# landrumb/ParlayANN

Measured on AMD Instinct MI355X. Metric: QPS @ recall@10>=0.95, SIFT-1M d=128 beam=64; achieved HBM GB/s vs roofline, higher is better.
Workload: dtype f16; 1 GPU; SIFT-1M-shaped batched beam search: 1000000x128 integer-valued fp32->f16 base, 10000 queries/step/GPU, beam=64 k=10 cut=1.35 start=0, prebuilt Vamana R=64 L=128 alpha=1.15 x2 passes (built on device); n=1000000, d=128, nq_per_gpu=10000, beam=64, k=10, parallelism=query-sharded x1, index replicated, no collective

## Files before the change

### parlayann_amd/csrc/api.hip

```cpp
#include <algorithm>
#include <chrono>
#include <cmath>
#include <cstring>
#include <mutex>
#include <vector>

#include "grouped_plan.h"
#include "host_staging.h"
#include "pann_internal.h"
#include "quant_device.h"

namespace pann {

static thread_local std::string g_err;
void set_error(const std::string& s) { g_err = s; }
int hip_fail(hipError_t e, const char* what) {
  g_err = std::string(what) + ": " + hipGetErrorString(e);
  return PANN_ERR_HIP;
}

constexpr size_t kAllocSlack = 4096;

int Workspace::ensure(size_t need) {
  if (need <= bytes) return PANN_OK;
// ... 440 lines not shown
uint64_t pann_index_size(const pann_index* idx) { return idx ? idx->ix.n : 0; }
uint32_t pann_index_dims(const pann_index* idx) { return idx ? idx->ix.d : 0; }
uint32_t pann_index_max_degree(const pann_index* idx) { return idx ? idx->ix.max_deg : 0; }
int pann_index_device(const pann_index* idx) { return idx ? idx->device : -1; }

int pann_index_set_exact_float_order(pann_index* idx, int on) {
  if (int rc = check_idx(idx, "pann_index_set_exact_float_order")) return rc;
  DeviceIndex& ix = idx->ix;
  const bool is_float = ix.dtype == PANN_F32 || ix.dtype == PANN_F16 || ix.dtype == PANN_BF16;
  if (on && is_float) { ix.exact = 1; ix.lpc = 4; ix.nch = ix.pstride / 64; }
  else { ix.exact = 0; choose_point_layout(ix.dbytes, &ix.lpc, &ix.nch); }
  return PANN_OK;
}

int pann_index_reserve_dropped(pann_index* idx, uint32_t cap) {
  if (int rc = check_idx(idx, "pann_index_reserve_dropped")) return rc;
  if (cap > (1u << 30)) { set_error("pann_index_reserve_dropped: capacity out of range"); return PANN_ERR_BAD_ARG; }
  if (cap > idx->dcap) idx->dcap = (cap + 63) / 64 * 64;
  return PANN_OK;
}
uint32_t pann_index_dropped_capacity(const pann_index* idx) { return idx ? idx->dcap : 0; }

int pann_index_set_graph(pann_index* idx, const uint32_t* graph) {
  if (int rc = check_idx(idx, "pann_index_set_graph")) return rc;
  if (!graph) { set_error("pann_index_set_graph: null graph"); return PANN_ERR_BAD_ARG; }
  DeviceGuard g(idx->device);
  return upload_graph_rows(idx, graph, idx->ix.n, nullptr);
}

int pann_index_update_rows(pann_index* idx, const uint32_t* row_ids, const uint32_t* rows, uint64_t m) {
  if (int rc = check_idx(idx, "pann_index_update_rows")) return rc;
  if (m && (!row_ids || !rows)) { set_error("pann_index_update_rows: null argument"); return PANN_ERR_BAD_ARG; }
  for (uint64_t i = 0; i < m; i++)
    if (row_ids[i] >= idx->ix.n) { set_error("ERROR: graph index out of range"); return PANN_ERR_BAD_ARG; }
  DeviceGuard g(idx->device);
  return upload_graph_rows(idx, rows, m, row_ids);
}

int pann_index_clear_graph(pann_index* idx) {
  if (int rc = check_idx(idx, "pann_index_clear_graph")) return rc;
  DeviceGuard g(idx->device);
  PANN_HIP(hipMemsetAsync(idx->ix.graph, 0xFF, (size_t)idx->ix.n * idx->ix.gstride * 4, idx->stream));
  if (idx->ix.gcode) PANN_HIP(hipMemsetAsync(idx->ix.gcode, 0xFF, (size_t)idx->ix.n * idx->ix.gstride * 2, idx->stream));
  PANN_HIP(hipStreamSynchronize(idx->stream));
  return PANN_OK;
}

int64_t pann_index_get_option(const pann_index* idx, const char* name) {
  if (!idx || !name) return -1;
  const std::string nm = name;
  if (nm == "forest_group") return idx->ix.forest_group;
  if (nm == "gt_pieces") return idx->gt_pieces;
  if (nm == "delete_range_keys") return idx->delete_range_keys;
  if (nm == "locality_order") return idx->ix.cell ? 1 : 0;
  if (nm == "filter_codes") return idx->ix.codes_valid ? 1 : 0;
  if (nm == "pinned_bytes") return (int64_t)(idx->pin_in.bytes + idx->pin_out.bytes);
  return -1;
}

int pann_index_set_stream(pann_index* idx, void* stream, int use_private) {
  if (int rc = check_idx(idx, "pann_index_set_stream")) return rc;
  DeviceGuard g(idx->device);
  PANN_HIP(hipStreamSynchronize(idx->stream));
  idx->stream = use_private ? idx->own_stream : (hipStream_t)stream;
  return PANN_OK;
}

int pann_index_set_option(pann_index* idx, const char* name, int64_t value) {
  if (int rc = check_idx(idx, "pann_index_set_option")) return rc;
  const std::string nm = name ? name : "";
  if (value < 0 || value > 0x7FFFFFFF) { set_error("pann_index_set_option: value out of range"); return PANN_ERR_BAD_ARG; }
  if (nm == "forest_group") idx->ix.forest_group = (uint32_t)value;
  else if (nm == "gt_pieces") idx->gt_pieces = (uint32_t)value;
  else if (nm == "delete_range_keys") idx->delete_range_keys = (uint32_t)value;
  else if (nm == "locality_pivots") { idx->locality_pivots = std::max<uint32_t>(2, std::min<uint32_t>((uint32_t)value, 65536)); idx->ix.cell = nullptr; idx->cells_state = idx->cells_state < 0 ? idx->cells_state : 0; }
  else if (nm == "locality_groups") { idx->locality_groups = (uint32_t)std::min<int64_t>(value, 4096); idx->ix.cell = nullptr; idx->cells_state = idx->cells_state < 0 ? idx->cells_state : 0; }
  else if (nm == "locality_order") {
    idx->ix.cell = nullptr;
    idx->ix.cell_min_batch = value == 2 ? 64u : 4096u;
    idx->cells_state = value ? ((idx->cell_buf.buf && idx->cells_state == 1) ? 1 : 0) : -2;
    if (idx->cells_state == 1) idx->ix.cell = idx->cell_buf.as<uint32_t>();
  }
  else if (nm == "filter_codes") {
    idx->ix.codes_valid = 0;
    idx->codes_state = value ? (idx->ix.rank16 ? 1 : 0) : -2;
  }
  else { set_error("pann_index_set_option: unknown option '" + nm + "'"); return PANN_ERR_BAD_ARG; }
  return PANN_OK;
}

int pann_index_get_graph(pann_index* idx, uint32_t* graph_out) {
  if (int rc = check_idx(idx, "pann_index_get_graph")) return rc;
  if (!graph_out) { set_error("pann_index_get_graph: null output"); return PANN_ERR_BAD_ARG; }
  DeviceGuard g(idx->device);
  DeviceIndex& ix = idx->ix;
  const size_t row_bytes = (size_t)(ix.max_deg + 1) * 4;
  const uint64_t slice = std::max<uint64_t>(1, (256ull << 20) / row_bytes);
  for (uint64_t r0 = 0; r0 < ix.n; r0 += slice) {
    const uint64_t cnt = std::min(slice, ix.n - r0);
    if (int rc = idx->graph_slab.ensure(cnt * row_bytes)) return rc;
    hipLaunchKernelGGL(graph_to_host_layout_kernel, dim3((uint32_t)cnt), dim3(64), 0, idx->stream,
                       ix.graph + r0 * (uint64_t)ix.gstride, idx->graph_slab.as<uint32_t>(), cnt, ix.max_deg, ix.gstride);
    PANN_HIP(hipGetLastError());
    PANN_HIP(hipMemcpyAsync(graph_out + r0 * (ix.max_deg + 1), idx->graph_slab.buf, cnt * row_bytes, hipMemcpyDeviceToHost, idx->stream));
    PANN_HIP(hipStreamSynchronize(idx->stream));
  }
  return PANN_OK;
}


static int masked_search_checks(const pann_index* idx, const PointFilter& F, uint64_t nq, const pann_query_params* qp, const pann_search_out* out) {
  if ((int64_t)out->out_k > qp->beam) { set_error("pann_batch_search_masked: out_k larger than the beam"); return PANN_ERR_BAD_ARG; }
  if (F.mode == MASK_BITMAP) { if (int rc = filter_checks(idx, "pann_batch_search_masked", F, nq)) return rc; }
  if (out->out_k > 64) { set_error("pann_batch_search_masked: out_k > 64 is not supported"); return PANN_ERR_UNSUPPORTED; }
  return PANN_OK;
}

static int search_common_checks(pann_index* idx, uint64_t nq, const pann_query_params* qp, const pann_search_out* out) {
  if (int rc = check_idx(idx, "pann_batch_search")) return rc;
  if (!qp || !out) { set_error("pann_batch_search: null params/out"); return PANN_ERR_BAD_ARG; }
  if (int rc = k_beam_check(qp)) return rc;
  (void)nq;
  return PANN_OK;
}

static int batch_search_dev_impl(pann_index* idx, const void* d_queries, const uint32_t* d_query_ids,
                                 uint64_t nq, uint64_t q_stride_bytes, const uint32_t* d_starts,
// ... 1897 lines not shown
```

### parlayann_amd/csrc/beam_search.hip

```cpp
#include <cstdio>
#include <cstdlib>
#include <vector>

#include "pann_device.h"

namespace pann {

#ifndef PANN_GU
#define PANN_GU 4
#endif
#ifndef PANN_GU_B128
#define PANN_GU_B128(LPC, NCH1) 4
#endif
#ifndef PANN_MINWAVES
#define PANN_MINWAVES 1
#endif
#ifndef PANN_B128_PAIR_CODES
#define PANN_B128_PAIR_CODES 1
#endif
#ifndef PANN_B64_PREFETCH
#define PANN_B64_PREFETCH 1
#endif
#ifndef PANN_MINWAVES_B64
#define PANN_MINWAVES_B64 7
// ... 69 lines not shown
}
template <bool HASH_LDS>
__device__ __forceinline__ void hstore(uint32_t* H, uint32_t s, uint32_t v) {
  if constexpr (HASH_LDS) H[s] = v;
  else __hip_atomic_store(H + s, v, __ATOMIC_RELAXED, PANN_PRIVATE_SCOPE);
}
template <bool HASH_LDS>
__device__ __forceinline__ void hsync() {
  if constexpr (!HASH_LDS) __builtin_amdgcn_s_waitcnt(0);
  PANN_WSYNC();
}

__device__ __forceinline__ uint32_t lower_bound_lds(const uint64_t* A, uint32_t n, uint64_t key) {
  uint32_t lo = 0, hi = n;
  while (lo < hi) {
    uint32_t mid = (lo + hi) >> 1;
    if (A[mid] < key) lo = mid + 1; else hi = mid;
  }
  return lo;
}

__device__ __forceinline__ uint32_t split_lds_index(uint32_t s, uint32_t hb) {
  return hb == 1 ? (s >> 1) : hb == 3 ? s : (s >> 2) * 3 + (s & 3);
}
struct LdsPart { uint8_t* base; uint32_t nslots; uint32_t p24; };
__device__ __forceinline__ uint32_t lds_part_load(const LdsPart& L, uint32_t i) {
  if (L.p24) {
    const uint32_t lo = reinterpret_cast<const uint16_t*>(L.base)[i];
    const uint32_t hi = (L.base + 2 * L.nslots)[i];
    return lo | (hi << 16);
  }
  return reinterpret_cast<const uint32_t*>(L.base)[i];
}
__device__ __forceinline__ void lds_part_store(const LdsPart& L, uint32_t i, uint32_t a) {
  if (L.p24) {
    reinterpret_cast<uint16_t*>(L.base)[i] = (uint16_t)a;
    (L.base + 2 * L.nslots)[i] = (uint8_t)(a >> 16);
  } else {
    reinterpret_cast<uint32_t*>(L.base)[i] = a;
  }
}
__device__ __forceinline__ void lds_part_clear(const LdsPart& L, int lane) {
  if (L.p24) {
    uint32_t* w = reinterpret_cast<uint32_t*>(L.base);
    for (uint32_t i = lane; i < (3 * L.nslots) / 4; i += PANN_WAVE) w[i] = 0xFFFFFFFFu;
  } else {
    uint32_t* w = reinterpret_cast<uint32_t*>(L.base);
    for (uint32_t i = lane; i < L.nslots; i += PANN_WAVE) w[i] = SENTINEL;
  }
}

template <bool HASH_LDS>
__device__ __forceinline__ bool filter_update(uint32_t* H, uint32_t hmask, bool active, uint32_t a, int lane,
                                              uint8_t* T = nullptr, uint32_t hb = 0, LdsPart Lp = LdsPart{nullptr, 0, 0}) {
  const uint32_t s = (uint32_t)hash64_2((uint64_t)a) & hmask;
  uint32_t old, w;
  const uint32_t hm = (1u << hb) - 1u;
  const bool in_hbm = hb != 3 && (s & hm) == hm;
  if constexpr (HASH_LDS) {
    old = active ? H[s] : 0u;
    PANN_WSYNC();
    if (active) H[s] = (uint32_t)lane;
    PANN_WSYNC();
    w = active ? H[s] : (uint32_t)lane;
  } else {
    __builtin_amdgcn_s_waitcnt(0);
    old = 0u;
    if (active) old = in_hbm ? __hip_atomic_load(H + (s >> hb), __ATOMIC_RELAXED, PANN_PRIVATE_SCOPE) : lds_part_load(Lp, split_lds_index(s, hb));
    const uint32_t t = s & 1023u;
    if (active) T[t] = (uint8_t)lane;
    PANN_WSYNC();
    w = active ? (uint32_t)T[t] : (uint32_t)lane;
  }
  uint64_t losers = __ballot(active && w != (uint32_t)lane);
  int prev = -1;
  bool last = true;
  while (losers) {
    const int L = __ffsll((unsigned long long)losers) - 1;
    const uint32_t sL = __builtin_amdgcn_readlane(s, L);
    const uint64_t grp = __ballot(active && s == sL);
    losers &= ~grp;
    if (active && s == sL) {
      const uint64_t below = grp & ((1ull << lane) - 1ull);
      prev = below ? 63 - __clzll((unsigned long long)below) : -1;
      last = (lane == 63) ? true : ((grp >> (lane + 1)) == 0ull);
    }
  }
  const uint32_t a_prev = __shfl(a, prev < 0 ? lane : prev);
  const bool seen = active && (prev >= 0 ? (a_prev == a) : (old == a));
  if constexpr (HASH_LDS) {
    PANN_WSYNC();
    if (active && last) H[s] = a;
    PANN_WSYNC();
  } else {
    if (active && last) {
      if (in_hbm) __hip_atomic_store(H + (s >> hb), a, __ATOMIC_RELAXED, PANN_PRIVATE_SCOPE);
      else lds_part_store(Lp, split_lds_index(s, hb), a);
    }
    PANN_WSYNC();
  }
  return seen;
}

struct FilterUndo { uint32_t s, old; bool wrote; };
__device__ __forceinline__ void code_store(uint8_t* P8, uint32_t* P4, uint32_t s, uint32_t code) {
  const uint32_t sh = (s & 7u) * 4u;
  P8[s] = (uint8_t)code;
  const uint32_t addr = (uint32_t)(uintptr_t)(P4 + (s >> 3));
  asm volatile("ds_mskor_b32 %0, %1, %2" ::"v"(addr), "v"(0xFu << sh), "v"((code >> 8) << sh) : "memory");
}
__device__ __forceinline__ void filter_undo_codes(uint8_t* P8, uint32_t* P4, const FilterUndo& u) {
  if (u.wrote) code_store(P8, P4, u.s, u.old);
  PANN_WSYNC();
}
__device__ __forceinline__ bool filter_update_codes(uint8_t* P8, uint32_t* P4, uint32_t hmask, bool active, uint32_t a, uint32_t code,
                                                    int lane, uint8_t* T, FilterUndo* undo = nullptr) {
  const uint32_t s = (uint32_t)hash64_2((uint64_t)a) & hmask;
  const uint32_t sh = (s & 7u) * 4u;
  uint32_t old = 0x1000u;
  if (active) old = (uint32_t)P8[s] | (((P4[s >> 3] >> sh) & 0xFu) << 8);
  const uint32_t t = s & 1023u;
  if (active) T[t] = (uint8_t)lane;
  PANN_WSYNC();
  const uint32_t w = active ? (uint32_t)T[t] : (uint32_t)lane;
  uint64_t losers = __ballot(active && w != (uint32_t)lane);
  int prev = -1;
  bool last = true;
  while (losers) {
    const int L = __ffsll((unsigned long long)losers) - 1;
    const uint32_t sL = __builtin_amdgcn_readlane(s, L);
    const uint64_t grp = __ballot(active && s == sL);
    losers &= ~grp;
    if (active && s == sL) {
      const uint64_t below = grp & ((1ull << lane) - 1ull);
      prev = below ? 63 - __clzll((unsigned long long)below) : -1;
      last = (lane == 63) ? true : ((grp >> (lane + 1)) == 0ull);
    }
  }
  const uint32_t a_prev = __shfl(a, prev < 0 ? lane : prev);
  const bool seen = active && (prev >= 0 ? (a_prev == a) : (old == code));
  if (undo) { undo->s = s; undo->old = old; undo->wrote = active && last; }
  if (active && last) code_store(P8, P4, s, code);
  PANN_WSYNC();
// ... 384 lines not shown
              }
              const uint64_t lm = __ballot(lost);
              if (lost) {
                const uint32_t at = ndrop + lanes_below(lm, lane);
                if (at < P.dcap) DL[at] = key; else atomicOr(P.status, 2u);
              }
              ndrop = min(ndrop + (uint32_t)__popcll(lm), P.dcap);
            }
            __builtin_amdgcn_s_waitcnt(0);
          }
          { uint64_t* t = F; F = NF; NF = t; uint8_t* tv = Fv; Fv = NFv; NFv = tv; }
          f = f_new;
          c = 0;
          PANN_WSYNC();
        }
      }
      PANN_STAMP(4);
      first = false;
    }

    const size_t qo = (size_t)qi * P.out.out_k;
    if constexpr (MASKED) {
      const uint64_t rkey = R.L[lane];
      const uint64_t fill = __ballot(rkey != KEY_INF);
      if (lane < (int)P.out.out_k) {
        const bool ok = rkey != KEY_INF;
        if (P.out.ids) P.out.ids[qo + lane] = ok ? key_id(rkey) : SENTINEL;
        if (P.out.dists) P.out.dists[qo + lane] = ok ? key_dist(rkey) : __builtin_inff();
      }
      if (lane == 0) {
        if (P.result_count) P.result_count[qi] = min((uint32_t)__popcll(fill), P.out.out_k);
        if (P.allowed_cmps) P.allowed_cmps[qi] = R.cmps;
      }
    } else {
    for (uint32_t j = lane; j < P.out.out_k; j += PANN_WAVE) {
      const bool ok = j < f;
      uint64_t key = 0ull;
      if (ok) key = F[j];
      if (P.out.ids) P.out.ids[qo + j] = ok ? key_id(key) : SENTINEL;
      if (P.out.dists) P.out.dists[qo + j] = ok ? key_dist(key) : __builtin_inff();
    }
    }
    PANN_STAMP_FLUSH(qi);
    if (lane == 0) {
      write_counters(P, qi, f, nvis, dcmps, degsum);
      if constexpr (FILTER) if (P.pruned_cmps) P.pruned_cmps[qi] = pcmps;
    }
    PANN_WSYNC();
    if constexpr (HASH_LDS) break;
    else slot = next_slot(P, lane);
  }
}

template <int DT, int METRIC, int LPC, bool NCH1, int MASKED = MASK_NONE>
__global__ void __launch_bounds__(PANN_WAVE, PANN_MINWAVES_B64) beam_search_b64_kernel(BSParams P) {
  const int lane = threadIdx.x;
  extern __shared__ __align__(16) uint8_t smem[];
  uint64_t* S = reinterpret_cast<uint64_t*>(smem);
  uint64_t* C = S + 64;
  uint8_t* Sv = reinterpret_cast<uint8_t*>(C + P.ccap);
  uint4* qlds = reinterpret_cast<uint4*>(Sv + 64);
  uint32_t* H = reinterpret_cast<uint32_t*>(qlds + (NCH1 ? 0 : P.nch * LPC));
  uint32_t* Pl = reinterpret_cast<uint32_t*>(S);

  const uint32_t hsize = 1u << P.bits, hmask = hsize - 1u;
  const uint32_t beam = P.beam;
  const uint32_t BIG_ORD = f2ord(2147483648.0f);
  const uint32_t qi = P.order ? P.order[blockIdx.x] : blockIdx.x;
  if (blockIdx.x >= P.prio_start) __builtin_amdgcn_s_setprio(3);

  for (uint32_t i = lane; i < hsize; i += PANN_WAVE) H[i] = SENTINEL;
  const int64_t self = P.query_ids ? (int64_t)P.query_ids[qi] : -1;
  const uint8_t* qrow = P.query_ids ? P.points + (uint64_t)self * P.pstride : P.queries + (uint64_t)qi * P.qstride;
  QReg<DT> qreg{};
  load_query<DT, LPC, NCH1>(qrow, P.dbytes, P.nch, qreg, qlds, lane);
  PANN_WSYNC();

  uint32_t f = 0, c = 0, nvis = 0, dcmps = P.nstarts, degsum = 0, ndrop = 0;
  uint64_t fkey = KEY_INF;
  uint32_t fflag = 0;
  uint64_t* DL = P.dropped + (size_t)qi * P.dcap;
  [[maybe_unused]] MaskedList R{reinterpret_cast<uint64_t*>(smem + P.rl_off), P.out.out_k ? KEY_INF : 0ull, 0u};
  [[maybe_unused]] const uint32_t thr_lane = P.out.out_k ? P.out.out_k - 1u : 0u;
  [[maybe_unused]] MaskSrc M{};
  if constexpr (MASKED) { M = mask_src<MASKED>(P, qi); R.L[lane] = KEY_INF; }
  PANN_STAMP_BEGIN();

  {
    const bool act = lane < (int)P.nstarts;
    const uint32_t a = act ? P.starts[(size_t)qi * P.starts_stride + lane] : 0u;
    (void)filter_update<true>(H, hmask, act, a, lane);
    [[maybe_unused]] uint32_t aword = 0u;
    if constexpr (MASKED) if (act) aword = mask_word<MASKED>(M, a);
    if (act) Pl[lane] = a;
    PANN_WSYNC();
    if constexpr (MASKED)
      c = gather_distances_masked<DT, METRIC, LPC, NCH1, 4, MASKED>(P, qreg, qlds, Pl, P.nstarts, 0xFFFFFFFFu, C, c, lane,
                                                            masked_note(act, (uint32_t)lane, a), aword, M, R, thr_lane);
    else
    c = gather_distances<DT, METRIC, LPC, NCH1, 4>(P, qreg, qlds, Pl, P.nstarts, 0xFFFFFFFFu, C, c, lane);
    PANN_WSYNC();
  }

  uint32_t pref_id = SENTINEL, pref_row = SENTINEL;
  bool first = true;
  for (;;) {
    bool do_merge = first;
    if (!first) {
      const uint64_t um = __ballot(lane < (int)f && fflag == 0);
      if (um == 0ull || nvis >= P.limit) break;
      const int cur_idx = __ffsll((unsigned long long)um) - 1;
      const bool more_unvisited = (um & (um - 1)) != 0ull;
      PANN_STAMP(0);
      const uint64_t cur_key = readlane64(fkey, cur_idx);
      const uint32_t cur = key_id(cur_key);
      if (lane == cur_idx) fflag = 1;
      if (lane == 0 && P.out.visited_cap) record_visit(P, qi, nvis, cur_key);
      nvis++;
      uint32_t cutoff_ord = BIG_ORD;
      if (f == beam) cutoff_ord = (uint32_t)(readlane64(fkey, (int)f - 1) >> 32);

      asm volatile("s_waitcnt vmcnt(0)" : "+v"(pref_row));
      const bool pref_hit = PANN_B64_PREFETCH && (pref_id == cur);
      const uint32_t pref_val = pref_row;
      pref_id = SENTINEL;
      if (PANN_B64_PREFETCH) {
        const uint64_t rest = um & (um - 1);
        if (rest) {
          pref_id = key_id(readlane64(fkey, __ffsll((unsigned long long)rest) - 1));
          const uint32_t* np = P.graph + (size_t)pref_id * P.gstride + min((uint32_t)lane, P.gstride - 1);
          asm volatile("global_load_dword %0, %1, off" : "=v"(pref_row) : "v"(np));
        }
      }

      const uint32_t* row = P.graph + (size_t)cur * P.gstride;
      for (uint32_t i0 = 0; i0 < P.gstride; i0 += PANN_WAVE) {
        const uint32_t i = i0 + lane;
        uint32_t a = SENTINEL;
        if (i0 == 0 && pref_hit) { if (i < P.gstride) a = pref_val; }
        else if (i < P.gstride) a = row[i];
        const bool act = (a != SENTINEL) && (i < P.degree_limit);
        const uint64_t am = __ballot(act);
        PANN_STAMP(1);
        if (am == 0ull) break;
        degsum += __popcll(am);
        const bool seen = filter_update<true>(H, hmask, act, a, lane);
        const bool keep = act && !seen && ((int64_t)a != self);
        const uint64_t km = __ballot(keep);
        const uint32_t m = __popcll(km);
        [[maybe_unused]] uint32_t aword = 0u;
        if constexpr (MASKED) if (keep) aword = mask_word<MASKED>(M, a);
        const uint32_t mypos = lanes_below(km, lane);
        if (keep) Pl[mypos] = a;
        dcmps += m;
        PANN_WSYNC();
        PANN_STAMP(2);
        if constexpr (MASKED) {
          if (m) c = gather_distances_masked<DT, METRIC, LPC, NCH1, PANN_GU, MASKED>(P, qreg, qlds, Pl, m, cutoff_ord, C, c, lane,
                                                                             masked_note(keep, mypos, a), aword, M, R, thr_lane);
        } else {
        if (m) c = gather_distances<DT, METRIC, LPC, NCH1, PANN_GU>(P, qreg, qlds, Pl, m, cutoff_ord, C, c, lane);
        }
        PANN_WSYNC();
        PANN_STAMP(3);
      }
      const bool skip = (c == 0) || (P.skip_enabled && c < beam / 8 && more_unvisited);
      do_merge = !skip;
    }
    if (do_merge) {
      const uint32_t f_old = f;
      const bool track = P.cut_enabled && !first;
      uint32_t lt = 0;
      for (uint32_t c0 = 0; c0 < c; c0 += PANN_WAVE) {
        const uint32_t cc = min(c - c0, (uint32_t)PANN_WAVE);
        const uint64_t ckey = (lane < (int)cc) ? C[c0 + lane] : KEY_INF;
        const bool fl = lane < (int)f;
        uint32_t myp = 0, rank_c = 0, below_f = 0;
        uint64_t live_mask = 0;
        const uint64_t vmask = __ballot(fl);
        const uint32_t cid = (uint32_t)ckey, fid = (uint32_t)fkey;
        for (uint32_t i = 0; i < cc; i++) {
          const uint64_t kk = readlane64(ckey, (int)i);
          const uint32_t kid = (uint32_t)kk;
          const bool g = kk < fkey;
          const uint64_t gtm = __ballot(g);
          const uint64_t eqm = __ballot(fid == kid);
          const uint64_t dupm = __ballot(cid == kid) & ((1ull << i) - 1ull);
          if (eqm == 0ull && dupm == 0ull) {
            live_mask |= 1ull << i;
            if (lane == (int)i) myp = f - (uint32_t)__popcll(gtm & vmask);
            rank_c += (kk < ckey) ? 1u : 0u;
            below_f += g ? 1u : 0u;
          }
        }
        const uint32_t nvalid = __popcll(live_mask);
        const bool clive = (lane < (int)cc) && ((live_mask >> lane) & 1ull);
        const uint32_t cpos = rank_c + myp, fpos = (uint32_t)lane + below_f;
        if (clive && cpos < beam) {
          uint32_t flag = 0u;
          for (uint32_t t = 0; t < ndrop; t++)
            flag |= (__hip_atomic_load(DL + t, __ATOMIC_RELAXED, PANN_PRIVATE_SCOPE) == ckey) ? 2u : 0u;
          S[cpos] = ckey; Sv[cpos] = (uint8_t)flag;
        }
        if (fl && fpos < beam) { S[fpos] = fkey; Sv[fpos] = (uint8_t)fflag; }
        if (track) {
          const bool lost = fl && fflag == 1u && fpos >= beam;
          const uint64_t lm = __ballot(lost);
          if (lost) {
            const uint32_t at = ndrop + lt + lanes_below(lm, lane);
            if (at < P.dcap) DL[at] = fkey; else atomicOr(P.status, 2u);
          }
          lt += __popcll(lm);
        }
        PANN_WSYNC();
        f = min(f + nvalid, beam);
        fkey = (lane < (int)f) ? S[lane] : KEY_INF;
        fflag = (lane < (int)f) ? (uint32_t)Sv[lane] : 0u;
        PANN_WSYNC();
      }
      uint32_t f_new = f;
      if (!first && P.cut_enabled && f_new > P.k) {
        const float dk = key_dist(readlane64(fkey, (int)P.k));
        const float thr = (float)(P.cut * (double)dk);
        const uint64_t thr_key = (uint64_t)f2ord(thr) << 32;
        const uint32_t ub = __popcll(__ballot(lane < (int)f_new && fkey <= thr_key));
        f_new = max(ub, f_old);
      }
      if (f_new == beam) {
        ndrop = 0;
      } else if (track) {
        const bool lost = lane >= (int)f_new && lane < (int)f && fflag == 1u;
        const uint64_t lm = __ballot(lost);
        if (lost) {
          const uint32_t at = ndrop + lt + lanes_below(lm, lane);
          if (at < P.dcap) DL[at] = fkey; else atomicOr(P.status, 2u);
        }
        lt += __popcll(lm);
        ndrop = min(ndrop + lt, P.dcap);
        if (lt) __builtin_amdgcn_s_waitcnt(0);
      }
      f = f_new;
      if (lane >= (int)f) { fkey = KEY_INF; fflag = 0u; }
      c = 0;
    }
    PANN_STAMP(4);
    first = false;
  }
  asm volatile("s_waitcnt vmcnt(0)" : "+v"(pref_row));

  const size_t qo = (size_t)qi * P.out.out_k;
  if constexpr (MASKED) {
    const uint64_t rkey = R.L[lane];
    const uint64_t fill = __ballot(rkey != KEY_INF);
    if (lane < (int)P.out.out_k) {
      const bool ok = rkey != KEY_INF;
      if (P.out.ids) P.out.ids[qo + lane] = ok ? key_id(rkey) : SENTINEL;
      if (P.out.dists) P.out.dists[qo + lane] = ok ? key_dist(rkey) : __builtin_inff();
    }
    if (lane == 0) {
      if (P.result_count) P.result_count[qi] = min((uint32_t)__popcll(fill), P.out.out_k);
      if (P.allowed_cmps) P.allowed_cmps[qi] = R.cmps;
    }
  } else
  if (lane < (int)P.out.out_k) {
    const bool ok = lane < (int)f;
    if (P.out.ids) P.out.ids[qo + lane] = ok ? key_id(fkey) : SENTINEL;
    if (P.out.dists) P.out.dists[qo + lane] = ok ? key_dist(fkey) : __builtin_inff();
  }
  PANN_STAMP_FLUSH(qi);
  if (lane == 0) write_counters(P, qi, f, nvis, dcmps, degsum);
}

template <int DT, int METRIC, int LPC, bool NCH1, bool HASH_LDS, bool CODES = false>
__global__ void __launch_bounds__(PANN_WAVE) beam_search_b128_kernel(BSParams P) {
  static_assert(!CODES || HASH_LDS, "the code table lives in LDS");
  constexpr int RB = 2;
  const int lane = threadIdx.x;
  extern __shared__ __align__(16) uint8_t smem[];
  uint64_t* S = reinterpret_cast<uint64_t*>(smem);
// ... 273 lines not shown
  PANN_STAMP_FLUSH(qi);

  const size_t qo = (size_t)qi * P.out.out_k;
#pragma unroll
  for (int r = 0; r < RB; r++) {
    const uint32_t j = lane + 64 * r;
    if (j < P.out.out_k) {
      const bool ok = j < f;
      if (P.out.ids) P.out.ids[qo + j] = ok ? key_id(fkey[r]) : SENTINEL;
      if (P.out.dists) P.out.dists[qo + j] = ok ? key_dist(fkey[r]) : __builtin_inff();
    }
  }
  if (lane == 0) write_counters(P, qi, f, nvis, dcmps, degsum);
  if constexpr (HASH_LDS) {
    break;
  } else {
    PANN_WSYNC();
    slot = next_slot(P, lane, slot);
  }
  }
}


void choose_point_layout(uint32_t dbytes, uint32_t* lpc, uint32_t* nch) {
  const uint32_t r64 = (dbytes + 63) / 64 * 64;
  if (const char* f = ab_env("PANN_FORCE_LPC")) {
    const uint32_t l = (uint32_t)atoi(f);
    if ((l == 4 || l == 8 || l == 16) && r64 % (l * 16) == 0 && r64 / (l * 16) > 1) { *lpc = l; *nch = r64 / (l * 16); return; }
  }
  if (r64 == 128) { *lpc = 8; *nch = 1; return; }
  if (r64 == 256) { *lpc = 16; *nch = 1; return; }
  if (r64 == 512) { *lpc = 32; *nch = 1; return; }
  if (r64 % 256 == 0) { *lpc = 16; *nch = r64 / 256; return; }
  if (r64 % 128 == 0) { *lpc = 8; *nch = r64 / 128; return; }
  *lpc = 4; *nch = r64 / 64;
}

static uint32_t filter_bits(int64_t beam) {
  double l = std::ceil(std::log2((double)beam * (double)beam)) - 2.0;
  int b = (int)l;
  return (uint32_t)(b < 10 ? 10 : b);
}

struct Plan {
  uint32_t bits, bcap, ccap, deg_eff, dcap, lds_bytes; bool hash_lds; uint32_t slots; bool b64; bool b128;
  bool b128_codes;
  bool b128_hbm;
  uint32_t hsplit;
  uint32_t p24;
  bool filter; uint32_t sk_lds_off;
  uint32_t rl_off;
  bool masked;
  bool by_labels;
};

constexpr bool masked_b64_fits(int dtype, uint32_t lpc, bool nch1) { return !(lpc == 8 && nch1) && !(dtype == PANN_BF16 && !nch1); }

static Plan make_plan(const DeviceIndex& ix, const SearchArgs& a) {
  Plan p;
  p.bits = filter_bits(a.beam);
  const uint32_t beam = (uint32_t)a.beam;
  p.bcap = (std::max<uint32_t>(beam, a.nstarts) + 63) / 64 * 64;
  int64_t dl = std::min<int64_t>(std::max<int64_t>(a.degree_limit, 0), (int64_t)ix.max_deg);
  p.deg_eff = (uint32_t)dl;
  p.ccap = (std::max<uint32_t>(beam / 8 + p.deg_eff, a.nstarts) + 63) / 64 * 64;
  p.dcap = std::max<uint32_t>(a.dcap, 64);
  const bool nch1 = layout_query_in_registers(ix);
  size_t fixed = (size_t)p.bcap * 8 * 2 + (size_t)p.ccap * 8 + (size_t)p.bcap * 2 +
                 (size_t)p.ccap * 2 + (nch1 ? 0 : (size_t)ix.nch * ix.lpc * 16);
  size_t hbytes = (size_t)4 << p.bits;
  p.hash_lds = (hbytes <= 16384) && (fixed + hbytes <= 64 * 1024);
  p.lds_bytes = (uint32_t)(fixed + (p.hash_lds ? hbytes : 1024));
  p.slots = 256 * 8;
  p.filter = a.filter != 0; p.sk_lds_off = 0;
  p.masked = a.masked != MASK_NONE; p.by_labels = a.masked == MASK_LABELS; p.rl_off = 0;
  const bool masked_b64 = p.hash_lds && p.bcap == 64 && masked_b64_fits(ix.dtype, ix.lpc, nch1);
  if (p.masked && !masked_b64) {
    p.b64 = p.b128 = p.b128_codes = p.b128_hbm = false; p.hsplit = 0; p.p24 = 0;
    p.rl_off = (p.lds_bytes + 15u) & ~15u;
    p.lds_bytes = p.rl_off + 1024;
    return p;
  }
  if (p.filter) {
    p.b64 = p.b128 = p.b128_codes = p.b128_hbm = false; p.hsplit = 0; p.p24 = 0;
    p.sk_lds_off = (p.lds_bytes + 15u) & ~15u;
    p.lds_bytes = p.sk_lds_off + ix.sk_stride;
    return p;
  }
  p.b64 = p.hash_lds && p.bcap == 64;
  if (p.b64) {
    p.ccap = (std::max<uint32_t>(beam / 8 + p.deg_eff, a.nstarts) + 7) / 8 * 8;
    p.lds_bytes = (uint32_t)(64 * 8 + (size_t)p.ccap * 8 + 64 + (nch1 ? 0 : (size_t)ix.nch * ix.lpc * 16) + hbytes);
    if (p.masked) { p.rl_off = (p.lds_bytes + 15u) & ~15u; p.lds_bytes = p.rl_off + 1024; }
  }
  p.b128 = p.hash_lds && p.bcap == 128 && a.nstarts <= 64;
  p.b128_hbm = false;
  p.b128_codes = p.b128 && p.bits == FILTER_CODE_BITS && ix.codes_valid && ix.gcode && ix.rank16 && ix.gstride <= PANN_WAVE;
  if (p.b128_codes) {
    p.ccap = (std::max<uint32_t>(beam / 8 + p.deg_eff, a.nstarts) + 7) / 8 * 8;
    p.hsplit = 0; p.p24 = 0;
    p.lds_bytes = (uint32_t)(128 * 8 + (size_t)p.ccap * 8 + 128 + (nch1 ? 0 : (size_t)ix.nch * ix.lpc * 16) + ((size_t)1 << p.bits) * 3 / 2);
  } else if (p.b128) {
    p.ccap = (std::max<uint32_t>(beam / 8 + p.deg_eff, a.nstarts) + 7) / 8 * 8;
    static const bool force_lds = ab_env("PANN_B128_LDS") != nullptr;
    p.b128_hbm = (hbytes > 8192) && a.nq > 2048 && !force_lds;
    p.hsplit = 0;
    if (p.b128_hbm) {
      static const char* sp = ab_env("PANN_B128_SPLIT");
      p.hsplit = sp ? (uint32_t)atoi(sp) : 1u;
      if (p.hsplit > 3) p.hsplit = 0;
      static const bool no24 = ab_env("PANN_B128_NO24") != nullptr;
      if (p.hsplit == 3 && (no24 || !(ix.n < 0xFFFFFFull))) p.hsplit = 1;
      p.hash_lds = false; p.slots = 256 * 32;
      p.p24 = (p.hsplit && ix.n < 0xFFFFFFull && !no24) ? 1u : 0u;
      hbytes = p.hsplit == 3 ? ((size_t)3 << p.bits)
             : p.hsplit ? (((size_t)1 << p.bits) - ((size_t)1 << (p.bits - p.hsplit))) * (p.p24 ? 3 : 4) : 0;
    }
    p.lds_bytes = (uint32_t)(128 * 8 + (size_t)p.ccap * 8 + 128 + (nch1 ? 0 : (size_t)ix.nch * ix.lpc * 16) + hbytes);
  }
  return p;
}

size_t search_workspace_bytes(const DeviceIndex& ix, const SearchArgs& a) {
  Plan p = make_plan(ix, a);
  size_t need = 256;
  need += (size_t)a.nq * p.dcap * 8;
  if (!p.hash_lds) need += ((size_t)std::min<uint64_t>(a.nq, p.slots) << p.bits) * 4;
  return need;
}

using SearchKernel = void (*)(BSParams);
static hipError_t launch_search(SearchKernel kern, const BSParams& P, const Plan& p, bool persistent, hipStream_t stream) {
  if (p.lds_bytes > 48 * 1024)
    (void)hipFuncSetAttribute(reinterpret_cast<const void*>(kern), hipFuncAttributeMaxDynamicSharedMemorySize, (int)p.lds_bytes);
  const uint32_t grid = persistent ? (uint32_t)std::min<uint64_t>(P.nq, p.slots) : P.nq;
  hipLaunchKernelGGL(kern, dim3(grid), dim3(PANN_WAVE), p.lds_bytes, stream, P);
  return hipGetLastError();
}

template <int DT, int METRIC, int LPC, bool NCH1, int MODE>
static SearchKernel masked_kernel(const Plan& p) {
  if (p.b64) {
    if constexpr (masked_b64_fits(DT, LPC, NCH1)) return beam_search_b64_kernel<DT, METRIC, LPC, NCH1, MODE>;
    else return nullptr;
  }
  if (p.hash_lds) return beam_search_kernel<DT, METRIC, LPC, NCH1, true, false, MODE>;
  return beam_search_kernel<DT, METRIC, LPC, NCH1, false, false, MODE>;
}

template <int DT, int METRIC, int LPC, bool NCH1>
static hipError_t launch_variant(const BSParams& P, const Plan& p, hipStream_t stream) {
  SearchKernel kern;
  if (p.filter) {
    if (p.hash_lds) kern = beam_search_kernel<DT, METRIC, LPC, NCH1, true, true>;
    else kern = beam_search_kernel<DT, METRIC, LPC, NCH1, false, true>;
  } else if (p.masked) {
    kern = p.by_labels ? masked_kernel<DT, METRIC, LPC, NCH1, MASK_LABELS>(p) : masked_kernel<DT, METRIC, LPC, NCH1, MASK_BITMAP>(p);
    if (!kern) return hipErrorInvalidValue;
  } else if (p.b64) {
    kern = beam_search_b64_kernel<DT, METRIC, LPC, NCH1>;
  } else if (p.b128_codes) {
    kern = beam_search_b128_kernel<DT, METRIC, LPC, NCH1, true, true>;
  } else if (p.b128) {
    if (p.b128_hbm) kern = beam_search_b128_kernel<DT, METRIC, LPC, NCH1, false>;
    else kern = beam_search_b128_kernel<DT, METRIC, LPC, NCH1, true>;
  } else if (p.hash_lds) {
    kern = beam_search_kernel<DT, METRIC, LPC, NCH1, true>;
  } else {
    kern = beam_search_kernel<DT, METRIC, LPC, NCH1, false>;
  }
  return launch_search(kern, P, p, !p.hash_lds, stream);
}

template <int DT, int METRIC>
static hipError_t launch_layout(const DeviceIndex& ix, const BSParams& P, const Plan& p, hipStream_t s) {
  if (layout_query_in_registers(ix)) {
    if (ix.lpc == 8) return launch_variant<DT, METRIC, 8, true>(P, p, s);
    if (ix.lpc == 16) return launch_variant<DT, METRIC, 16, true>(P, p, s);
    if (ix.lpc == 32) return launch_variant<DT, METRIC, 32, true>(P, p, s);
  }
  if (ix.lpc == 4) return launch_variant<DT, METRIC, 4, false>(P, p, s);
  if (ix.lpc == 8) return launch_variant<DT, METRIC, 8, false>(P, p, s);
  if (ix.lpc == 16) return launch_variant<DT, METRIC, 16, false>(P, p, s);
  return hipErrorInvalidValue;
}

int launch_beam_search(const DeviceIndex& ix, const SearchArgs& a, void* ws, size_t ws_bytes,
                       hipStream_t stream) {
  if (a.nq == 0) return PANN_OK;
  if (a.nq > 0xFFFFFFF0ull) { set_error("pann_batch_search: nq too large"); return PANN_ERR_BAD_ARG; }
  if (a.beam <= 0 || a.beam > 65536) { set_error("pann_batch_search: beam out of range [1,65536]"); return PANN_ERR_BAD_ARG; }
  if (a.nstarts == 0) {
    set_error("beam search expects at least one start point"); return PANN_ERR_BAD_ARG;
  }
  if ((int64_t)a.nstarts > a.beam) { set_error("pann_batch_search: more start points than beam"); return PANN_ERR_BAD_ARG; }
  if (a.out.out_k > (uint64_t)a.beam) {
    set_error("Error: beam search parameter Q same size or smaller than k"); return PANN_ERR_BAD_ARG;
  }
  if ((a.queries == nullptr) == (a.query_ids == nullptr)) {
    set_error("pann_batch_search: exactly one of queries / query_ids must be given"); return PANN_ERR_BAD_ARG;
  }
  if (a.filter) {
    if (!ix.sketch || !sketch_kind_ok(ix.sk_kind)) { set_error("pann_batch_search_filtered: no sketch attached to the index"); return PANN_ERR_BAD_ARG; }
    if ((a.queries != nullptr) != (a.sketch_queries != nullptr)) {
      set_error("pann_batch_search_filtered: sketch_queries go with queries, and only with them"); return PANN_ERR_BAD_ARG;
    }
    if (a.sketch_queries && (a.sq_stride < sketch_row_bytes(ix.sk_kind, ix.d) || a.sq_stride % 8 != 0 || (uintptr_t)a.sketch_queries % 8 != 0)) {
      set_error("pann_batch_search_filtered: sketch query stride smaller than a sketch row, or rows not 8-byte aligned"); return PANN_ERR_BAD_ARG;
    }
  }
  if (a.masked && a.filter) { set_error("pann_batch_search_masked: the sketch filter has no masked form"); return PANN_ERR_UNSUPPORTED; }
  if (a.masked == MASK_LABELS && (!a.labels || !a.preds || a.pred_stride > 1 || !pred_kind_known(a.pred_kind))) {
    set_error("pann_batch_search_labeled: labels, predicates of a known kind and a predicate stride of 0 or 1 are needed"); return PANN_ERR_BAD_ARG;
// ... 77 lines not shown
```

### parlayann_amd/csrc/pann_internal.h

```cpp
#pragma once
#include <hip/hip_runtime.h>
#include <stdint.h>
#include <stdlib.h>
#include <algorithm>
#include <string>

#include "../../include/pann.h"

namespace pann {

constexpr uint32_t SENTINEL = 0xFFFFFFFFu;

#ifdef PANN_AB
inline const char* ab_env(const char* name) { return getenv(name); }
#else
inline const char* ab_env(const char*) { return nullptr; }
#endif

inline bool is_4bit_dtype(int dtype) { return dtype == PANN_U4 || dtype == PANN_I4; }
inline const char* dtype_name(int dtype) {
  switch (dtype) {
    case PANN_U8: return "PANN_U8"; case PANN_I8: return "PANN_I8"; case PANN_F32: return "PANN_F32"; case PANN_F16: return "PANN_F16";
    case PANN_BF16: return "PANN_BF16"; case PANN_U4: return "PANN_U4"; case PANN_I4: return "PANN_I4";
  }
  return "unknown dtype";
}
inline uint32_t esize_of(int dtype) {
  switch (dtype) { case PANN_U8: case PANN_I8: return 1; case PANN_F16: case PANN_BF16: return 2; case PANN_F32: return 4; }
  return 0;
}
inline bool dtype_known(int dtype) { return esize_of(dtype) != 0 || is_4bit_dtype(dtype); }
inline uint64_t row_bytes_of(int dtype, uint64_t d) { return is_4bit_dtype(dtype) ? (d + 1) / 2 : d * esize_of(dtype); }

struct DeviceIndex {
  uint8_t* points = nullptr;
  uint32_t* graph = nullptr;
  uint64_t n = 0;
  uint32_t d = 0;
  int dtype = 0, metric = 0;
  uint32_t esize = 0;
  uint32_t dbytes = 0;
  uint32_t pstride = 0;
  uint32_t lpc = 0;
  uint32_t nch = 0;
  uint32_t exact = 0;
  uint32_t max_deg = 0;
  uint32_t gstride = 0;
  uint32_t forest_group = 0;
  const uint16_t* rank16 = nullptr;
  uint16_t* gcode = nullptr;
  uint32_t codes_valid = 0;
  const uint32_t* cell = nullptr;
  uint32_t cell_min_batch = 4096;
  const uint8_t* sketch = nullptr;
  uint32_t sk_stride = 0;
  int sk_kind = -1;
  uint32_t sk_as_written = 0;
  const uint32_t* labels = nullptr;
};

inline bool layout_query_in_registers(const DeviceIndex& ix) { return ix.nch == 1 && ix.lpc != 4; }
inline size_t query_lds_bytes(const DeviceIndex& ix) { return layout_query_in_registers(ix) ? 0 : (size_t)ix.nch * ix.lpc * 16; }

enum { MASK_NONE = 0, MASK_BITMAP = 1, MASK_LABELS = 2 };
inline bool pred_kind_known(int kind) { return kind == PANN_PRED_ANY || kind == PANN_PRED_MATCH || kind == PANN_PRED_RANGE; }

struct SearchArgs {
  const uint8_t* queries; uint64_t qstride;
  const uint32_t* query_ids;
  uint64_t nq;
  const uint32_t* starts; uint32_t nstarts;
  int starts_per_query = 0;
  int64_t k, beam, limit, degree_limit; double cut;
  uint32_t dcap = 256;
  const uint32_t* order = nullptr;
  pann_search_out out;
  int filter = 0;
  const uint8_t* sketch_queries = nullptr;
  uint64_t sq_stride = 0;
  uint32_t* pruned_cmps = nullptr;
  int masked = 0;
  const uint32_t* allow = nullptr;
  uint64_t allow_stride = 0;
  uint32_t* result_count = nullptr;
  uint32_t* allowed_cmps = nullptr;
  const uint32_t* labels = nullptr;
  const pann_label_pred* preds = nullptr;
  uint32_t pred_stride = 0;
  int pred_kind = 0;
};

struct PointFilter {
  enum { SHARED, PER_QUERY, TABLE };
  int mode = MASK_NONE, layout = SHARED;
  uint64_t count = 1;
  const uint32_t* allow = nullptr; uint64_t stride = 0;
  const uint32_t* labels = nullptr; int kind = 0; const pann_label_pred* preds = nullptr;
  const uint32_t* group = nullptr; bool dev = false;
  static PointFilter bitmap(const uint32_t* allow, uint64_t stride, uint64_t nq, bool dev) {
    PointFilter f; f.mode = MASK_BITMAP; f.allow = allow; f.stride = stride; f.dev = dev;
    if (stride) { f.layout = PER_QUERY; f.count = nq; }
// ... 184 lines not shown
```

Before: 7.435 million queries/s.

## Add LDS victim cache to skip distance recomputation for hash-evicted candidates in b64 search

Adds a small direct-mapped LDS victim table holding node ids evicted from the visited hash filter in the beam-64 kernel. When a neighbor hits this table while the beam is full, its key is looked up in the frontier or candidate lists and re-inserted without fetching the vector or recomputing the distance. It is on by default via a new index option, and it costs extra LDS per block, possible occupancy loss, and extra per-iteration ballots and readlane loops.

```diff
diff --git a/parlayann_amd/csrc/api.hip b/parlayann_amd/csrc/api.hip
--- a/parlayann_amd/csrc/api.hip
+++ b/parlayann_amd/csrc/api.hip
@@ -516,6 +516,7 @@
   if (nm == "forest_group") return idx->ix.forest_group;
   if (nm == "gt_pieces") return idx->gt_pieces;
   if (nm == "delete_range_keys") return idx->delete_range_keys;
+  if (nm == "b64_seen") return idx->ix.b64_seen;
   if (nm == "locality_order") return idx->ix.cell ? 1 : 0;
   if (nm == "filter_codes") return idx->ix.codes_valid ? 1 : 0;
   if (nm == "pinned_bytes") return (int64_t)(idx->pin_in.bytes + idx->pin_out.bytes);
@@ -537,6 +538,7 @@
   if (nm == "forest_group") idx->ix.forest_group = (uint32_t)value;
   else if (nm == "gt_pieces") idx->gt_pieces = (uint32_t)value;
   else if (nm == "delete_range_keys") idx->delete_range_keys = (uint32_t)value;
+  else if (nm == "b64_seen") idx->ix.b64_seen = value ? 1u : 0u;
   else if (nm == "locality_pivots") { idx->locality_pivots = std::max<uint32_t>(2, std::min<uint32_t>((uint32_t)value, 65536)); idx->ix.cell = nullptr; idx->cells_state = idx->cells_state < 0 ? idx->cells_state : 0; }
   else if (nm == "locality_groups") { idx->locality_groups = (uint32_t)std::min<int64_t>(value, 4096); idx->ix.cell = nullptr; idx->cells_state = idx->cells_state < 0 ? idx->cells_state : 0; }
   else if (nm == "locality_order") {
diff --git a/parlayann_amd/csrc/beam_search.hip b/parlayann_amd/csrc/beam_search.hip
--- a/parlayann_amd/csrc/beam_search.hip
+++ b/parlayann_amd/csrc/beam_search.hip
@@ -145,7 +145,8 @@
 
 template <bool HASH_LDS>
 __device__ __forceinline__ bool filter_update(uint32_t* H, uint32_t hmask, bool active, uint32_t a, int lane,
-                                              uint8_t* T = nullptr, uint32_t hb = 0, LdsPart Lp = LdsPart{nullptr, 0, 0}) {
+                                              uint8_t* T = nullptr, uint32_t hb = 0, LdsPart Lp = LdsPart{nullptr, 0, 0},
+                                              uint32_t* victim = nullptr) {
   const uint32_t s = (uint32_t)hash64_2((uint64_t)a) & hmask;
   uint32_t old, w;
   const uint32_t hm = (1u << hb) - 1u;
@@ -182,6 +183,7 @@
   const uint32_t a_prev = __shfl(a, prev < 0 ? lane : prev);
   const bool seen = active && (prev >= 0 ? (a_prev == a) : (old == a));
   if constexpr (HASH_LDS) {
+    if (victim) *victim = (active && last && old != SENTINEL && old != a) ? old : SENTINEL;
     PANN_WSYNC();
     if (active && last) H[s] = a;
     PANN_WSYNC();
@@ -672,8 +674,12 @@
   }
 }
 
-template <int DT, int METRIC, int LPC, bool NCH1, int MASKED = MASK_NONE>
+enum { B64_SEEN = 3 };
+template <int DT, int METRIC, int LPC, bool NCH1, int MODE = MASK_NONE>
 __global__ void __launch_bounds__(PANN_WAVE, PANN_MINWAVES_B64) beam_search_b64_kernel(BSParams P) {
+  constexpr int MASKED = (MODE == MASK_BITMAP || MODE == MASK_LABELS) ? MODE : MASK_NONE;
+  constexpr int VN = MODE == B64_SEEN ? (int)B64_SEEN_N : 0;
+  static_assert((B64_SEEN_N & (B64_SEEN_N - 1)) == 0 && B64_SEEN_N >= 128, "V: a power of two of whole words per lane");
   const int lane = threadIdx.x;
   extern __shared__ __align__(16) uint8_t smem[];
   uint64_t* S = reinterpret_cast<uint64_t*>(smem);
@@ -686,6 +692,10 @@
   const uint32_t hsize = 1u << P.bits, hmask = hsize - 1u;
   const uint32_t beam = P.beam;
   const uint32_t BIG_ORD = f2ord(2147483648.0f);
+  constexpr uint32_t VSHIFT = VN ? (uint32_t)__builtin_ctz((unsigned)(VN ? VN : 1)) : 0u;
+  [[maybe_unused]] uint16_t* V = reinterpret_cast<uint16_t*>(H + hsize);
+  [[maybe_unused]] bool v_ok = true;
+  if constexpr (VN != 0) for (uint32_t i = lane; i < VN / 2; i += PANN_WAVE) reinterpret_cast<uint32_t*>(V)[i] = 0xFFFFFFFFu;
   const uint32_t qi = P.order ? P.order[blockIdx.x] : blockIdx.x;
   if (blockIdx.x >= P.prio_start) __builtin_amdgcn_s_setprio(3);
 
@@ -764,15 +774,44 @@
         PANN_STAMP(1);
         if (am == 0ull) break;
         degsum += __popcll(am);
-        const bool seen = filter_update<true>(H, hmask, act, a, lane);
-        const bool keep = act && !seen && ((int64_t)a != self);
+        [[maybe_unused]] uint32_t victim = SENTINEL;
+        bool seen;
+        if constexpr (VN != 0) seen = filter_update<true>(H, hmask, act, a, lane, nullptr, 0, LdsPart{nullptr, 0, 0}, &victim);
+        else seen = filter_update<true>(H, hmask, act, a, lane);
+        bool keep = act && !seen && ((int64_t)a != self);
+        if constexpr (VN != 0) {
+          dcmps += __popcll(__ballot(keep));
+          if (f == beam && v_ok && cutoff_ord <= BIG_ORD && c <= PANN_WAVE) {
+            const bool hit = keep && V[a & (VN - 1)] == (uint16_t)(a >> VSHIFT);
+            uint64_t hm = __ballot(hit);
+            if (hm) {
+              const uint64_t pkey = lane < (int)c ? C[lane] : KEY_INF;
+              const uint32_t fid = (uint32_t)fkey, pid = (uint32_t)pkey;
+              while (hm) {
+                const int l = __ffsll((unsigned long long)hm) - 1;
+                hm &= hm - 1;
+                const uint32_t al = __builtin_amdgcn_readlane(a, l);
+                const uint64_t inf = __ballot(fid == al), inc = __ballot(pid == al);
+                uint64_t key = KEY_INF;
+                if (inf) key = readlane64(fkey, __ffsll((unsigned long long)inf) - 1);
+                else if (inc) key = readlane64(pkey, __ffsll((unsigned long long)inc) - 1);
+                if ((uint32_t)(key >> 32) < cutoff_ord) {
+                  if (lane == 0) C[c] = key;
+                  c++;
+                }
+              }
+              keep = keep && !hit;
+            }
+          }
+          if (victim != SENTINEL) V[victim & (VN - 1)] = (uint16_t)(victim >> VSHIFT);
+        }
         const uint64_t km = __ballot(keep);
         const uint32_t m = __popcll(km);
         [[maybe_unused]] uint32_t aword = 0u;
         if constexpr (MASKED) if (keep) aword = mask_word<MASKED>(M, a);
         const uint32_t mypos = lanes_below(km, lane);
         if (keep) Pl[mypos] = a;
-        dcmps += m;
+        if constexpr (VN == 0) dcmps += m;
         PANN_WSYNC();
         PANN_STAMP(2);
         if constexpr (MASKED) {
@@ -845,6 +884,7 @@
         const uint64_t thr_key = (uint64_t)f2ord(thr) << 32;
         const uint32_t ub = __popcll(__ballot(lane < (int)f_new && fkey <= thr_key));
         f_new = max(ub, f_old);
+        if constexpr (VN != 0) if (f_new <= P.k) v_ok = false;
       }
       if (f_new == beam) {
         ndrop = 0;
@@ -1224,6 +1264,7 @@
   uint32_t rl_off;
   bool masked;
   bool by_labels;
+  uint32_t seen_n;
 };
 
 constexpr bool masked_b64_fits(int dtype, uint32_t lpc, bool nch1) { return !(lpc == 8 && nch1) && !(dtype == PANN_BF16 && !nch1); }
@@ -1246,6 +1287,7 @@
   p.slots = 256 * 8;
   p.filter = a.filter != 0; p.sk_lds_off = 0;
   p.masked = a.masked != MASK_NONE; p.by_labels = a.masked == MASK_LABELS; p.rl_off = 0;
+  p.seen_n = 0;
   const bool masked_b64 = p.hash_lds && p.bcap == 64 && masked_b64_fits(ix.dtype, ix.lpc, nch1);
   if (p.masked && !masked_b64) {
     p.b64 = p.b128 = p.b128_codes = p.b128_hbm = false; p.hsplit = 0; p.p24 = 0;
@@ -1264,6 +1306,13 @@
     p.ccap = (std::max<uint32_t>(beam / 8 + p.deg_eff, a.nstarts) + 7) / 8 * 8;
     p.lds_bytes = (uint32_t)(64 * 8 + (size_t)p.ccap * 8 + 64 + (nch1 ? 0 : (size_t)ix.nch * ix.lpc * 16) + hbytes);
     if (p.masked) { p.rl_off = (p.lds_bytes + 15u) & ~15u; p.lds_bytes = p.rl_off + 1024; }
+    bool seen = ix.b64_seen != 0;
+    if (const char* sv = ab_env("PANN_B64_SEEN")) seen = atoi(sv) != 0;
+    const bool cut_monotone = !(a.k > 0 && ix.metric == PANN_L2) || a.cut >= 0.0;
+    if (!p.masked && seen && cut_monotone && ix.n <= (uint64_t)0xFFFF * B64_SEEN_N) {
+      p.seen_n = B64_SEEN_N;
+      p.lds_bytes += B64_SEEN_N * 2;
+    }
   }
   p.b128 = p.hash_lds && p.bcap == 128 && a.nstarts <= 64;
   p.b128_hbm = false;
@@ -1330,7 +1379,7 @@
     kern = p.by_labels ? masked_kernel<DT, METRIC, LPC, NCH1, MASK_LABELS>(p) : masked_kernel<DT, METRIC, LPC, NCH1, MASK_BITMAP>(p);
     if (!kern) return hipErrorInvalidValue;
   } else if (p.b64) {
-    kern = beam_search_b64_kernel<DT, METRIC, LPC, NCH1>;
+    kern = p.seen_n ? beam_search_b64_kernel<DT, METRIC, LPC, NCH1, B64_SEEN> : beam_search_b64_kernel<DT, METRIC, LPC, NCH1>;
   } else if (p.b128_codes) {
     kern = beam_search_b128_kernel<DT, METRIC, LPC, NCH1, true, true>;
   } else if (p.b128) {
diff --git a/parlayann_amd/csrc/pann_internal.h b/parlayann_amd/csrc/pann_internal.h
--- a/parlayann_amd/csrc/pann_internal.h
+++ b/parlayann_amd/csrc/pann_internal.h
@@ -10,6 +10,7 @@
 namespace pann {
 
 constexpr uint32_t SENTINEL = 0xFFFFFFFFu;
+constexpr uint32_t B64_SEEN_N = 512;
 
 #ifdef PANN_AB
 inline const char* ab_env(const char* name) { return getenv(name); }
@@ -47,6 +48,7 @@
   uint32_t max_deg = 0;
   uint32_t gstride = 0;
   uint32_t forest_group = 0;
+  uint32_t b64_seen = 1;
   const uint16_t* rank16 = nullptr;
   uint16_t* gcode = nullptr;
   uint32_t codes_valid = 0;
```

New measurement: 7.733 million queries/s (median of 6 runs). +4.0%, better.
